# 3dhumangan/3DHumanGAN

Measured on AMD Instinct MI355X. Metric: generator images/sec at 512^2, higher is better.
Workload: dtype f32 in/out, f32 accumulate; contractions field f16x2 / synthesis f16x2 (x2 = f16 product + block-scaled fp6 cross terms, x3 = three f16/bf16 products); 1 GPU; BASELINE cfg 3: MAP3DBN512 generator-only forward, 512x512 out, 96x96 rays x 64 samples, hidden 256, batch 16/GPU, mixed, random-init weights, procedural SMPL-like pose; global_batch=16, parallelism=batch-sharded replicas x1 (no collective)

## Files before the change

### 3dhumangan_amd/_lib.py

```python
import ctypes as C
import os

_HERE = os.path.dirname(os.path.abspath(__file__))
LIB_PATH = os.path.join(_HERE, "csrc", "libh3d.so")

_lib = None


class H3DError(RuntimeError):
    pass


class FieldParams(C.Structure):
    _fields_ = [("w_coord", C.c_void_p), ("b_coord", C.c_void_p), ("w_geo", C.c_void_p), ("b_geo", C.c_void_p),
                ("w_film", C.c_void_p * 4), ("b_film", C.c_void_p * 4), ("w_sigma", C.c_void_p),
                ("b_sigma", C.c_void_p), ("w_color", C.c_void_p), ("b_color", C.c_void_p), ("w_rgb", C.c_void_p),
                ("b_rgb", C.c_void_p), ("w_feat", C.c_void_p), ("b_feat", C.c_void_p)]


_p, _i, _l, _f = C.c_void_p, C.c_int, C.c_int64, C.c_float
_SIGNATURES = {
    "h3d_version": (C.c_int, []),
    "h3d_last_error": (C.c_char_p, []),
    "h3d_device_info": (C.c_int, [C.POINTER(C.c_int), C.c_char_p, _i]),
    "h3d_ray_integrate": (C.c_int, [_p, _p, _p, _p, _p, _p, _l, _i, _i, _i, _i, _i, _p]),
    "h3d_ray_setup": (C.c_int, [_p, _p, _p, _p, _p, _p, _i, _i, _i, _i, _f, _f, _p]),
    "h3d_geo_features": (C.c_int, [_p, _p, _p, _p, _p, _p, _p, _i, _l, _i, _i, _i, _p]),
    "h3d_nearest_vertex": (C.c_int, [_p, _p, _p, _i, _l, _i, _p]),
    "h3d_mesh_sort_bytes": (C.c_int64, [_i, _i]),
    "h3d_mesh_sort": (C.c_int, [_p, _p, _i, _i, _p]),
    "h3d_geo_features_sorted": (C.c_int, [_p, _p, _p, _p, _p, _p, _p, _i, _l, _i, _i, _i, _p]),
    "h3d_nearest_vertex_sorted": (C.c_int, [_p, _p, _p, _i, _l, _i, _p]),
    "h3d_nearest_vertex_sorted_rays": (C.c_int, [_p, _p, _p, _i, _i, _i, _i, _i, _p]),
    "h3d_render_fused_x2_geo": (C.c_int, [_p] * 7 + [_i, _i] + [_p] * 8 + [_i, _i, _i, _i, _i, _f, _i, _i, _i, _p]),
    "h3d_render_fused_x3_geo": (C.c_int, [_p] * 7 + [_i, _i] + [_p] * 8 + [_i, _i, _i, _i, _i, _f, _i, _i, _i, _p]),
    "h3d_render_fused_x2_geo_ref": (C.c_int, [_p] * 7 + [_i, _i] + [_p] * 8 + [_i, _i, _i, _i, _i, _f, _i, _i, _i, _f, _f, _p, _p, _i, _p]),
    "h3d_render_fused_x3_geo_units": (C.c_int, [_p] * 7 + [_i, _i] + [_p] * 8 + [_i, _i, _i, _i, _i, _f, _i, _i, _i, _p, _p, _i, _p]),
    "h3d_field_pack_size": (C.c_int64, [_i, _i]),
    "h3d_field_pack": (C.c_int, [C.POINTER(FieldParams), _i, _i, _p]),
    "h3d_neural_field": (C.c_int, [_p, _p, _p, _p, _p, _p, _p, _i, _l, _i, _i, _i, _f, _p]),
    "h3d_render_fused": (C.c_int, [_p, _p, _p, _p, _p, _p, _p, _p, _p, _p, _p, _i, _i, _i, _i, _i, _i, _f, _i, _i,
                                   _i, _p]),
    "h3d_field_pack_x3_size": (C.c_int64, [_i, _i]),
    "h3d_field_pack_x3": (C.c_int, [C.POINTER(FieldParams), _i, _i, _p]),
    "h3d_field_pack_x3_device": (C.c_int, [C.POINTER(FieldParams), _i, _i, _p, _p]),
    "h3d_field_x3_layout": (C.c_int, [_i, _i, C.POINTER(C.c_int64), _i]),
    "h3d_neural_field_x3": (C.c_int, [_p, _p, _p, _p, _p, _p, _p, _i, _l, _i, _i, _i, _f, _p]),
    "h3d_render_fused_x3": (C.c_int, [_p, _p, _p, _p, _p, _p, _p, _p, _p, _p, _p, _i, _i, _i, _i, _i, _i, _f, _i,
                                      _i, _i, _p]),
    "h3d_conv_x3_tiling": (C.c_int, [_i, _i, C.POINTER(C.c_int)]),
    "h3d_conv_x3_pack": (C.c_int, [_p, _p, _i, _i, _i, _i, _p]),
    "h3d_conv_x3_pack_f16": (C.c_int, [_p, _p, _i, _i, _i, _i, _p]),
# ... 172 lines not shown
```

### 3dhumangan_amd/csrc/field_x3.hip

```cpp
#include "x3_common.hpp"
#include "field_pack.hpp"
#include "composite.hpp"
#include <string.h>
#include <math.h>
#include <stdio.h>
#include <algorithm>
#include <type_traits>

using namespace h3d;

namespace {

typedef F16::vec8 half8;
typedef F16::vec2 half2v;
typedef float f32x2 __attribute__((ext_vector_type(2)));

constexpr float kSA = 1.f;
constexpr float kSIn = 64.f;
constexpr int kLookF = 2;
constexpr int kValuF2 = 0;
constexpr int kValuF = 4;

enum { ST_COORD = 0, ST_GEO, ST_FILM0, ST_FILM1, ST_FILM2, ST_FILM3, ST_COLOR, ST_COUNT };
enum { W_COORD = 0, W_F0A, W_GEO, W_F0B, W_F1, W_F2, W_F3, W_COLOR, W_FEAT, W_COUNT };
// ... 53 lines not shown
    int Hd, F, geo_stride, S, clamp_mode, last_back, white_back;
    int R, log2S;
    int n_groups;
    float input_scaler;
    LayoutX3 L;
    const int* nn_index;
    const float* joints;
    const float* vertices;
    const float* tpose;
    const float* vertex_ik;
    int V, legacy_mode;
    int* ref_list;
    int* ref_count;
    int ref_cap, ref_mode;
    float ref_eps, ref_scale;
};

constexpr int kHeadPad = 64;
constexpr int kJointRows = 40;

__device__ __forceinline__ unsigned split2_act(float a, float b, unsigned& lo) {
    const half2v h2 = __builtin_convertvector(f32x2{a, b}, half2v);
    const float fa = (float)h2.x, fb = (float)h2.y;
    float la, lb;
    asm("v_sub_f32 %0, %1, %2" : "=v"(la) : "v"(a), "v"(fa));
    asm("v_sub_f32 %0, %1, %2" : "=v"(lb) : "v"(b), "v"(fb));
    lo = __builtin_bit_cast(unsigned, __builtin_convertvector(f32x2{la, lb}, half2v));
    return __builtin_bit_cast(unsigned, h2);
}

// ... 133 lines not shown
        const half8 tail[1] = {xl[KS]};
        gemm_x2_roll<NT, KS, KS3, 2 * NT + 1, NT, SWAP, kLookF, kValuF2, ZERO>(dst, xh, b6, tail, ring, hook, pre);
    } else {
        gemm_x3_roll<F16, NT, KSG, 2 * NT + 1, SWAP, kLookF, kValuF, ZERO>(dst, xh, xl, ring, hook);
    }
}

template <int NT, int KSG, typename RING, typename NEXT>
__device__ __forceinline__ void input_layer(f32x16 (&dst)[NT], const half8 (&ih)[2], const half8 (&il)[2], RING& ring, NEXT& next) {
    gemm_x3_roll<F16, NT, KSG, 2, false, kLookF, kValuF, true>(dst, ih, il, ring, [&](auto gc) __attribute__((always_inline)) {
        next_tile0<NT / 2, KSG - 1, decltype(gc)::value>(next);
    });
}


constexpr int kRingX2 = 8;

template <int NT, bool FUSED, bool X2, bool GEOIN = false>
__global__ __launch_bounds__(256, 1) void field_x3_kernel(Args A) {
    constexpr int KS = 2 * NT;
    extern __shared__ __attribute__((aligned(16))) float smem[];
    const LayoutX3& L = A.L;
    const int HdP = L.HdP;
    float* tab0 = smem;
    float* tfeat0 = tab0 + ST_COUNT * 2 * HdP;
    float* scratch = tfeat0 + HdP;
    float* joint0 = scratch + 4 * 64;
    unsigned char* head0 = reinterpret_cast<unsigned char*>(joint0 + (GEOIN ? kJointRows * 4 : 0));
    unsigned char* ring_lds = head0 + 4 * ((X2 ? 3 : 2) * KS * 32 + kHeadPad);

    const int t = threadIdx.x, lane = t & 63;
    const int wave = __builtin_amdgcn_readfirstlane(t >> 6);
    const int m = lane & 31, h = lane >> 5;
    const int b = blockIdx.y;
// ... 49 lines not shown
    __syncthreads();

    const float* __restrict__ head_inv = reinterpret_cast<const float*>(A.blob + L.head_inv);
    const float* __restrict__ head_b = reinterpret_cast<const float*>(A.blob + L.head_b);
    float inv_f = invs[W_FEAT];
    float hi0 = head_inv[0], hi1 = head_inv[1], hi2 = head_inv[2], hi3 = head_inv[3];
    float hb0 = head_b[0], hb1 = head_b[1], hb2 = head_b[2], hb3 = head_b[3];
    asm volatile("" : "+v"(inv_f), "+v"(hi0), "+v"(hi1), "+v"(hi2), "+v"(hi3), "+v"(hb0), "+v"(hb1), "+v"(hb2), "+v"(hb3));
    float* wl_lds = scratch + wave * 64;

    const int unit = FUSED ? (S > 32 ? S : 32) : 32;
    const int steps = unit / 32;
    const int seglen = FUSED ? (S < 32 ? S : 32) : 32;
    typedef typename std::conditional<X2, WeightRing<NT, kRingX2, 1>, WeightRing<NT>>::type Ring;
    Ring ring;
    ring.init(A.blob + L.w[0], ring_lds, L.stages, wave, lane);
    int n_groups = A.n_groups;
    if constexpr (FUSED) {
        if (A.ref_mode == 2) n_groups = (ref_units + 3) >> 2;
    }
    asm volatile("" : "+s"(n_groups));
    int ref_mode = FUSED ? A.ref_mode : 0;
    float ref_eps = A.ref_eps, ref_scale = A.ref_scale;
    typedef __attribute__((address_space(1))) int* gi32;
    gi32 ref_list = (gi32)A.ref_list + (int64_t)b * A.ref_cap, ref_count = (gi32)A.ref_count + b;
    int ref_cap = A.ref_cap;
    asm volatile("" : "+v"(ref_mode), "+v"(ref_eps), "+v"(ref_scale), "+v"(ref_list), "+v"(ref_count), "+v"(ref_cap));
    typedef const __attribute__((address_space(1))) float* gcf;
    typedef __attribute__((address_space(1))) float* gf;
    typedef const __attribute__((address_space(1))) int* gci;
    gcf a_points = (gcf)A.points, a_geo = (gcf)A.geo, a_dirs = (gcf)A.dirs, a_z = (gcf)A.z_vals, a_noise = (gcf)A.noise;
    gf a_feats = (gf)A.feats, a_depth = (gf)A.depth, a_weights = (gf)A.weights, a_out = (gf)A.out;
    gci a_nn = (gci)A.nn_index;
    gcf a_vik = (gcf)A.vertex_ik, a_tpose = (gcf)A.tpose, a_verts = (gcf)A.vertices;
    asm volatile("" : "+v"(a_points), "+v"(a_geo), "+v"(a_dirs), "+v"(a_z), "+v"(a_noise), "+v"(a_feats), "+v"(a_depth),
                      "+v"(a_weights), "+v"(a_out));
    if constexpr (GEOIN) asm volatile("" : "+v"(a_nn), "+v"(a_vik), "+v"(a_tpose), "+v"(a_verts));

#pragma unroll 1
    for (int ug = blockIdx.x; ug < n_groups; ug += gridDim.x) {
    int64_t uidx = (int64_t)ug * 4 + wave;
    if constexpr (FUSED) {
        if (ref_mode == 2) {
            const int slot = ug * 4 + wave;
            uidx = slot < ref_units ? (int64_t)__builtin_amdgcn_readfirstlane(ref_list[slot < ref_units ? slot : 0]) : N;
        }
    }
    const int64_t u0 = uidx * unit;
    const int64_t unit_ray = (int64_t)b * A.R + uidx;
    float smax = 0.f;
    auto ray_of = [&](int64_t nn) -> int64_t { return A.log2S < 0 ? unit_ray : (int64_t)b * A.R + (nn >> A.log2S); };

    RayCarry carry;
    float rgbacc = 0.f;
    float rayacc[NT];
#pragma unroll
    for (int i = 0; i < NT; ++i) rayacc[i] = 0.f;

    f32x16 X[NT], Y[NT];

    for (int si = 0; si < steps; ++si) {
        const int64_t n0 = u0 + (int64_t)si * 32;
        const int64_t n = n0 + m;
        const bool ok = n < N;
        const int64_t gi = (int64_t)b * N + (ok ? n : N - 1);
        const bool last_step = si == steps - 1;
        int opaque = 0;
        asm volatile("" : "+s"(opaque));
        const float* tab = tab0 + opaque;
// ... 118 lines not shown
            if (ok && h == 0) a_weights[gi] = w;
            if (h == 0) { wl_lds[m] = w; wl_lds[32 + m] = bg; }
            if (ref_mode == 1 && last_step) {
                float rmax = smax;
                for (int off = 1; off < seglen; off <<= 1) rmax = fmaxf(rmax, __shfl_xor(rmax, off, 32));
                const bool ill = last_abs >= 0.f && last_abs <= ref_eps * fmaxf(rmax, ref_scale);
                if (__any(ill)) {
                    if (lane == 0) {
                        const int slot = __hip_atomic_fetch_add(ref_count, 1, __ATOMIC_RELAXED, __HIP_MEMORY_SCOPE_AGENT);
                        if (slot < ref_cap) ref_list[slot] = (int)uidx;
                    }
                }
            }
        }

        layer<NT, KS, true, true, true, X2>(Y, xh, xl, b6, ring, p_col, none, hacc, head_lds, lane);
        pin_agpr<NT>(Y);
        float rgb[3];
        {
            const float c0 = __shfl(hacc[1], m, 64), c1 = __shfl(hacc[2], m, 64), c2 = __shfl(hacc[3], m, 64);
            rgb[0] = 1.f / (1.f + expf(-(c0 * hi1 + hb1)));
            rgb[1] = 1.f / (1.f + expf(-(c1 * hi2 + hb2)));
            rgb[2] = 1.f / (1.f + expf(-(c2 * hi3 + hb3)));
        }
        f32x16 (&acc)[NT] = Y;
        if (!FUSED) {
            if (ok && h == 0) {
                a_out[gi * (F + 4) + 0] = rgb[0];
                a_out[gi * (F + 4) + 1] = rgb[1];
                a_out[gi * (F + 4) + 2] = rgb[2];
            }
// ... 26 lines not shown
                    const int64_t ray = ray_of(n);
                    a_feats[ray * C + sl] = mine + (A.white_back ? bg : 0.f);
                }
            }
            __builtin_amdgcn_fence(__ATOMIC_RELEASE, "wavefront");
            __builtin_amdgcn_wave_barrier();
            float wr[16], wsum[4];
#pragma unroll
            for (int rg = 0; rg < 4; ++rg) {
                const f32x4 w4 = ld4(wl_lds + rg * 8 + 4 * h);
                wr[rg * 4 + 0] = w4.x; wr[rg * 4 + 1] = w4.y; wr[rg * 4 + 2] = w4.z; wr[rg * 4 + 3] = w4.w;
                wsum[rg] = (w4.x + w4.y) + (w4.z + w4.w);
            }
            const float wtot = (wsum[0] + wsum[1]) + (wsum[2] + wsum[3]);
            const float back = A.white_back ? wl_lds[32] : 0.f;
            gf fout = a_feats + ray_of(n0) * C + 3 + m;
            gf frg[4];
            float brg[4];
            bool okrg[4];
#pragma unroll
            for (int rg = 0; rg < 4; ++rg) {
                const int64_t n_first = n0 + rg * 8;
                okrg[rg] = h == 0 && n_first < N;
                frg[rg] = a_feats + ray_of(okrg[rg] ? n_first : n0) * C + 3 + m;
                brg[rg] = A.white_back ? wl_lds[32 + rg * 8] : 0.f;
            }
            const bool store_ray = last_step && h == 0 && n0 < N;
            const int g8 = S >> 3;
            const bool long_rays = S >= 32;
#pragma unroll
            for (int nt = 0; nt < NT; ++nt) {
                const int nn = nt * 32 + m;
                const bool okn = nn < F;
                const float bias = tfeat[okn ? nn : 0];
                pin1(acc[nt]);
                float s4[4];
#pragma unroll
                for (int rg = 0; rg < 4; ++rg) {
                    float s = acc[nt][rg * 4 + 0] * wr[rg * 4 + 0];
                    s = fmaf(acc[nt][rg * 4 + 1], wr[rg * 4 + 1], s);
                    s = fmaf(acc[nt][rg * 4 + 2], wr[rg * 4 + 2], s);
                    s4[rg] = fmaf(acc[nt][rg * 4 + 3], wr[rg * 4 + 3], s);
                }
                if (long_rays) {
                    float tot = fmaf((s4[0] + s4[1]) + (s4[2] + s4[3]), inv_f, bias * wtot);
                    tot += __shfl_xor(tot, 32, 64);
                    rayacc[nt] += tot;
                    if (store_ray && okn) fout[nt * 32] = rayacc[nt] + back;
                } else {
#pragma unroll
                    for (int rg = 0; rg < 4; ++rg) {
                        if (rg % g8 != 0) continue;
                        float sv = fmaf(s4[rg], inv_f, bias * wsum[rg]);
                        if (g8 == 2) sv += fmaf(s4[rg + 1 < 4 ? rg + 1 : 3], inv_f, bias * wsum[rg + 1 < 4 ? rg + 1 : 3]);
                        sv += __shfl_xor(sv, 32, 64);
                        if (okn && okrg[rg]) frg[rg][nt * 32] = sv + brg[rg];
                    }
                }
                __builtin_amdgcn_sched_barrier(0);
            }
            __builtin_amdgcn_wave_barrier();
        }
    }
    }
    ring.drain();
}

size_t lds_bytes(const LayoutX3& L, bool geoin = false) {
    return sizeof(float) * ((size_t)ST_COUNT * 2 * L.HdP + L.HdP + 4 * 64 + (geoin ? kJointRows * 4 : 0)) +
           (size_t)4 * (L.head_planes * L.KS * 32 + kHeadPad) + (L.head_planes == 3 ? kRingX2 : kWeightRingDepth) * (size_t)L.NT * 2048;
}

template <int NT, bool FUSED, bool X2, bool GEOIN = false>
int launch_one(Args A, int B, int64_t groups, hipStream_t st) {
    H3D_ALLOW_MAX_LDS((field_x3_kernel<NT, FUSED, X2, GEOIN>));
    A.n_groups = (int)groups;
    int64_t per_sample = h3d::persistent_wgs(groups, B, 4);
    if (A.ref_mode == 2) per_sample = std::max<int64_t>(1, std::min<int64_t>((A.ref_cap + 3) / 4, 8));
    h3d::pre_launch();
    hipLaunchKernelGGL((field_x3_kernel<NT, FUSED, X2, GEOIN>), dim3((unsigned)per_sample, (unsigned)B), dim3(256), lds_bytes(A.L, GEOIN), st, A);
    return h3d::launch_status(FUSED ? (X2 ? "h3d_render_fused_x2" : "h3d_render_fused_x3") : (X2 ? "h3d_neural_field_x2" : "h3d_neural_field_x3"));
}

template <bool FUSED>
int launch(const Args& A, int B, int64_t groups, hipStream_t st) {
    if constexpr (FUSED) {
        if (A.nn_index) {
            const bool x2 = A.L.head_planes == 3;
            if (A.L.NT == 4) return x2 ? launch_one<4, true, true, true>(A, B, groups, st) : launch_one<4, true, false, true>(A, B, groups, st);
            if (A.L.NT == 8) return x2 ? launch_one<8, true, true, true>(A, B, groups, st) : launch_one<8, true, false, true>(A, B, groups, st);
        }
    }
    if (A.L.head_planes == 3) {
        switch (A.L.NT) {
            case 4: return launch_one<4, FUSED, true>(A, B, groups, st);
            case 8: return launch_one<8, FUSED, true>(A, B, groups, st);
            default: break;
        }
    }
    switch (A.L.NT) {
        case 4: return launch_one<4, FUSED, false>(A, B, groups, st);
        case 8: return launch_one<8, FUSED, false>(A, B, groups, st);
        default:
// ... 258 lines not shown
    const float *joints, *vertices, *tpose, *vertex_ik;
    int V, legacy_mode;
};
struct RefIn {
    int mode;
    float eps, scale;
    int* list;
    int* count;
    int cap;
};

static int render_fused_x(bool x2, const void* packed, const float* points, const float* geo, const float* dirs,
                          const float* freq, const float* phase, const float* z_vals, const float* noise,
                          float* feats, float* depth, float* weights, int B, int R, int S, int Hd, int F,
                          int geo_stride, float input_scaler, int clamp_mode, int last_back, int white_back,
                          h3d_stream_t stream, const GeoIn* gin = nullptr, const RefIn* ref = nullptr) {
    const int64_t N = (int64_t)R * S;
    if (ref) {
        H3D_REQUIRE(ref->list && ref->count && ref->cap >= 1 && ref->cap <= 65536, "h3d_render_fused_x*: refinement list / count / cap=%d", ref->cap);
        H3D_REQUIRE(ref->mode == 2 || (ref->eps >= 0.f && ref->scale >= 0.f), "h3d_render_fused_x2_*_ref: eps and scale must be >= 0");
    }
    if (gin) {
        H3D_REQUIRE(gin->nn_index && gin->joints && gin->vertices && gin->tpose && gin->vertex_ik, "h3d_render_fused_x*_geo: null pointer");
        H3D_REQUIRE(gin->V >= 1 && h3d::aligned16(gin->vertex_ik), "h3d_render_fused_x*_geo: V=%d, vertex_ik must be 16-byte aligned", gin->V);
        geo = points;
        geo_stride = 31;
    }
    int rc = check_x3(packed, points, geo, freq, phase, B, N, Hd, F, geo_stride);
    if (rc) return rc;
    H3D_REQUIRE(z_vals && feats && depth && weights, "h3d_render_fused_x3: null pointer");
    H3D_REQUIRE(clamp_mode == 0 || clamp_mode == 1, "h3d_render_fused_x3: clamp_mode must be 0 (relu) or 1 (softplus)");
    H3D_REQUIRE(R >= 0 && S >= 1, "h3d_render_fused_x3: bad R=%d S=%d", R, S);
    const bool ok_s = (S >= 8 && S <= 32 && (S & (S - 1)) == 0) || (S > 32 && S % 32 == 0);
    if (!ok_s) {
        h3d::set_error("h3d_render_fused_x3: S=%d unsupported (needs 8, 16, 32 or a multiple of 32)", S);
        return H3D_EUNSUPPORTED;
    }
    if (B == 0 || N == 0) return H3D_OK;
    Args A{};
    A.blob = static_cast<const unsigned char*>(packed);
    A.points = points; A.geo = geo; A.dirs = dirs; A.freq = freq; A.phase = phase;
    A.z_vals = z_vals; A.noise = noise; A.feats = feats; A.depth = depth; A.weights = weights;
    A.N = N; A.Hd = Hd; A.F = F; A.geo_stride = geo_stride; A.S = S; A.input_scaler = input_scaler;
    A.clamp_mode = clamp_mode; A.last_back = last_back; A.white_back = white_back;
    A.R = R;
    A.log2S = -1;
    if (S <= 32) { A.log2S = 0; while ((1 << A.log2S) < S) ++A.log2S; }
    A.L = make_layout(Hd, F, x2);
    if (gin) {
        A.nn_index = gin->nn_index; A.joints = gin->joints; A.vertices = gin->vertices; A.tpose = gin->tpose;
        A.vertex_ik = gin->vertex_ik; A.V = gin->V; A.legacy_mode = gin->legacy_mode;
    }
    const int unit = S > 32 ? S : 32;
    const int64_t units = (N + unit - 1) / unit;
    const int64_t groups = (units + 3) / 4;
    H3D_REQUIRE(groups < (int64_t(1) << 31), "h3d_render_fused_x3: too many rays");
    if (ref) {
        A.ref_mode = ref->mode; A.ref_eps = ref->eps; A.ref_scale = ref->scale; A.ref_list = ref->list; A.ref_count = ref->count;
        A.ref_cap = ref->cap;
// ... 55 lines not shown
    return render_fused_x(true, packed, points, nullptr, dirs, freq, phase, z_vals, noise, feats, depth, weights, B, R, S, Hd, F, 31,
                          input_scaler, clamp_mode, last_back, white_back, stream, &g, &r);
}
extern "C" int h3d_render_fused_x3_geo_units(const void* packed, const float* points, const int32_t* nn_index, const float* joints,
                                             const float* vertices, const float* tpose_vertices, const float* vertex_ik, int V,
                                             int legacy_mode, const float* dirs, const float* freq, const float* phase,
                                             const float* z_vals, const float* noise, float* feats, float* depth, float* weights,
                                             int B, int R, int S, int Hd, int F, float input_scaler, int clamp_mode, int last_back,
                                             int white_back, const int32_t* ref_list, const int32_t* ref_count, int ref_cap,
                                             h3d_stream_t stream) {
    const GeoIn g{nn_index, joints, vertices, tpose_vertices, vertex_ik, V, legacy_mode};
    const RefIn r{2, 0.f, 0.f, const_cast<int32_t*>(ref_list), const_cast<int32_t*>(ref_count), ref_cap};
    return render_fused_x(false, packed, points, nullptr, dirs, freq, phase, z_vals, noise, feats, depth, weights, B, R, S, Hd, F, 31,
                          input_scaler, clamp_mode, last_back, white_back, stream, &g, &r);
}
```

### 3dhumangan_amd/lib/generators/map3d_generator.py

```python
import math
import os

import torch
import torch.nn as nn

from ... import _lib
from ..._stages import stage
from ..components import smpl
from ..components.ops.bias_act import bias_act
from . import volume_rendering as vr
from .differentiable import synthesis_forward
from .modsynth_pack import ModSynthesisPlan
from .style_input_pack import StyleInputPlan
from .synthesis_pack import SynthesisPlan


def normalize_2nd_moment(x, dim=1, eps=1e-8):
    return x * (x.square().mean(dim=dim, keepdim=True) + eps).rsqrt()


def _consume_camera_rng(sample_dist, batch, device):
    if sample_dist in ("uniform", "spherical_uniform"):
        torch.rand((batch, 1), device=device), torch.rand((batch, 1), device=device)
    elif sample_dist in ("normal", "gaussian"):
# ... 394 lines not shown
            feats, depths, weights = self._render_hierarchical(freq, phase, mesh, pts, z_vals, frame, S if fine_steps is None else int(fine_steps),
                                                               engine, lock_view_dependence, scaler, integ, nerf_noise, noise_coarse, fine_u, noise)
        else:
            noise = _integration_noise(noise, (B, R, S, 1), nerf_noise, dev)
            with stage(self, "geo_features"):
                if route == "fused_geo":
                    vik = smpl.vertex_inverse_transforms(c["fk_matrices"], c["lbs_weights"])
                    nn_index = smpl.nearest_vertex(pts, c["vertices"], ray_shape=(render_height, render_width, S))
                else:
                    geo = self.get_geo_features(pts, *mesh)
            dirs = None if lock_view_dependence else vr.ray_directions_world(focals, c["cam2world_matrices"], res, S)
            if route == "fused_geo":
                with stage(self, "render_fused"):
                    feats, depths, weights = nf.render_geo(pts, freq, phase, nn_index, *mesh[:3], vik, dirs, z_vals, S,
                                                           legacy_mode=self.legacy_mode, input_scaler=scaler, noise=noise,
                                                           precision=engine, **integ)
            elif route == "fused":
                with stage(self, "render_fused"):
                    feats, depths, weights = nf.render(pts, freq, phase, geo, dirs, z_vals, S, input_scaler=scaler, noise=noise,
                                                       precision=engine, **integ)
            else:
                with stage(self, "neural_field"):
                    field = nf(pts, freq, phase, geo, dirs, input_scaler=scaler, differentiable=differentiable, precision=engine)
                with stage(self, "ray_integrate"):
                    feats, depths, weights = vr.ray_integration(field.reshape(B, R, S, -1), z_vals, noise_std=0, noise=noise,
                                                                consume_rng=False, **integ)
        rgb_render = (feats[..., :3] * 2 - 1).reshape(B, render_height, render_width, 3).permute(0, 3, 1, 2)
        return rgb_render, feats[..., 3:], depths, weights, None

    def _render_hierarchical(self, freq, phase, mesh, pts, z_vals, frame, Sf, engine, lock_view_dependence, scaler, integ, nerf_noise,
                             noise_coarse, fine_u, noise):
# ... 178 lines not shown
```

### 3dhumangan_amd/lib/implicit_funcitions/modulated.py

```python
import ctypes
import math
import os
from typing import NamedTuple, Optional

import torch
import torch.nn as nn

from ... import _lib
from ..generators.volume_rendering import _CLAMP


class _Engine(NamedTuple):
    name: str
    pack_size: str
    pack: str
    device_pack: Optional[str]
    field: str
    render: str
    render_geo: Optional[str]
    tile: int
    tier: tuple


_ENGINES = {e.name: e for e in (
# ... 176 lines not shown
        pts, dirs, fr, ph, (z, nz, feats, depth, weights, mode) = self._prepare(input, ray_directions, frequencies, phase_shifts,
                                                                                 z_vals, num_steps, noise, clamp_mode)
        geo = geo_feature.contiguous().float()
        B, R, S = z.shape
        blob = self.packed_weights(pts.device, precision)
        rc = getattr(_lib.load(), eng.render)(_lib.ptr(blob), _lib.ptr(pts), _lib.ptr(geo), _lib.ptr(dirs), _lib.ptr(fr), _lib.ptr(ph),
                                              _lib.ptr(z), _lib.ptr(nz), _lib.ptr(feats), _lib.ptr(depth), _lib.ptr(weights), B, R, S,
                                              self.hidden_dim, self.feature_dim, geo.shape[-1], float(input_scaler), mode,
                                              int(bool(last_back)), int(bool(white_back)), *eng.tier, _lib.stream_handle())
        _lib.check(rc, "h3d_render_fused")
        return feats, depth, weights

    @torch.no_grad()
    def render_geo(self, input, frequencies, phase_shifts, nn_index, skeletons, vertices, tpose_vertices, vertex_ik,
                   ray_directions, z_vals, num_steps, legacy_mode=False, input_scaler=1., noise=None, clamp_mode="relu",
                   last_back=False, white_back=False, precision=None):
        _lib.need_cuda(input, frequencies, phase_shifts, nn_index, skeletons, vertices, tpose_vertices, vertex_ik,
                       ray_directions, z_vals, noise)
        eng = self._engine(precision)
        if eng.render_geo is None:
            raise ValueError(f"field engine {eng.name} has no fused render with in-kernel geometry")
        B, N, _ = input.shape
        idx = nn_index.contiguous()
        if idx.dtype != torch.int32 or tuple(idx.shape) != (B, N):
            raise ValueError("nn_index must be int32 [B, N]")
        sk, vt = skeletons.contiguous().float(), vertices.contiguous().float()
        tv, vik = tpose_vertices.contiguous().float(), vertex_ik.contiguous().float()
        if sk.shape[1:] != (24, 3) or vik.shape[1:] != (vt.shape[1], 16) or tv.shape != vt.shape:
            raise ValueError("skeletons [B,24,3], vertices / tpose_vertices [B,V,3], vertex_ik [B,V,16] expected")
        pts, dirs, fr, ph, (z, nz, feats, depth, weights, mode) = self._prepare(input, ray_directions, frequencies, phase_shifts,
                                                                                 z_vals, num_steps, noise, clamp_mode)
        _, R, S = z.shape
        blob = self.packed_weights(pts.device, precision)
        lib = _lib.load()
        common = lambda b: (_lib.ptr(b), _lib.ptr(pts), _lib.ptr(idx), _lib.ptr(sk), _lib.ptr(vt), _lib.ptr(tv), _lib.ptr(vik),
                            vt.shape[1], int(bool(legacy_mode)), _lib.ptr(dirs), _lib.ptr(fr), _lib.ptr(ph), _lib.ptr(z), _lib.ptr(nz),
                            _lib.ptr(feats), _lib.ptr(depth), _lib.ptr(weights), B, R, S, self.hidden_dim, self.feature_dim,
                            float(input_scaler), mode, int(bool(last_back)), int(bool(white_back)))
        if eng.name == "f16x2" and self.refine_last_sample:
            cap = self.refine_capacity
            buf = self._refine_buf
            if buf is None or buf[0].device != pts.device or buf[0].shape != (B, cap):
                buf = (torch.zeros(B, cap, dtype=torch.int32, device=pts.device), torch.zeros(B, dtype=torch.int32, device=pts.device))
                self._refine_buf = buf
            blob3 = self.packed_weights(pts.device, "f16x3")
            scale = self._sigma_scale(pts.device)
            rc = lib.h3d_render_fused_x2_geo_ref(*common(blob), float(self.refine_eps), scale, _lib.ptr(buf[0]), _lib.ptr(buf[1]), cap,
                                                 _lib.stream_handle())
            rc = rc or lib.h3d_render_fused_x3_geo_units(*common(blob3), _lib.ptr(buf[0]), _lib.ptr(buf[1]), cap, _lib.stream_handle())
        else:
            rc = getattr(lib, eng.render_geo)(*common(blob), _lib.stream_handle())
        _lib.check(rc, "h3d_render_fused_geo")
        return feats, depth, weights

    def _sigma_scale(self, device):
        w = self.sigma_layer.weight
        key = (w.data_ptr(), w._version, str(device))
        if self._sigma_scale_cache is None or self._sigma_scale_cache[0] != key:
            self._sigma_scale_cache = (key, float(w.detach().float().norm()))
        return self._sigma_scale_cache[1]

    def refined_units(self):
        return None if self._refine_buf is None else self._refine_buf[1]
```

### include/h3d.h

```cpp
#ifndef H3D_H
#define H3D_H

#include <stdint.h>

#ifdef __cplusplus
extern "C" {
#endif

#define H3D_VERSION 101

#define H3D_OK            0
#define H3D_EINVAL       -1
#define H3D_EUNSUPPORTED -2
#define H3D_ELAUNCH      -3

typedef void* h3d_stream_t;

int h3d_version(void);
const char* h3d_last_error(void);
int h3d_device_info(int* n_cu, char* name, int name_len);

int h3d_ray_integrate(const float* field, const float* z_vals, const float* noise,
                      float* feats, float* depth, float* weights,
                      int64_t n_rays, int S, int C,
// ... 139 lines not shown
int h3d_render_fused_x2_geo_ref(const void* packed, const float* points, const int32_t* nn_index, const float* joints,
                                const float* vertices, const float* tpose_vertices, const float* vertex_ik, int V,
                                int legacy_mode, const float* dirs, const float* freq, const float* phase,
                                const float* z_vals, const float* noise, float* feats, float* depth, float* weights,
                                int B, int R, int S, int Hd, int F, float input_scaler, int clamp_mode, int last_back,
                                int white_back, float ref_eps, float ref_scale, int32_t* ref_list, int32_t* ref_count,
                                int ref_cap, h3d_stream_t stream);
int h3d_render_fused_x3_geo_units(const void* packed, const float* points, const int32_t* nn_index, const float* joints,
                                  const float* vertices, const float* tpose_vertices, const float* vertex_ik, int V,
                                  int legacy_mode, const float* dirs, const float* freq, const float* phase,
                                  const float* z_vals, const float* noise, float* feats, float* depth, float* weights,
                                  int B, int R, int S, int Hd, int F, float input_scaler, int clamp_mode, int last_back,
                                  int white_back, const int32_t* ref_list, const int32_t* ref_count, int ref_cap,
                                  h3d_stream_t stream);

int64_t h3d_field_pack_x3t_size(int Hd, int F);
int h3d_field_pack_x3t(const h3d_field_params* p, int Hd, int F, void* blob );
int h3d_field_pack_x2t(const h3d_field_params* p, int Hd, int F, void* blob );
int h3d_field_x3t_layout(int Hd, int F, int64_t* out, int n_out);
int h3d_neural_field_x3t(const void* packed, const float* points, const float* geo, const float* dirs,
                         const float* freq, const float* phase, float* out,
                         int B, int64_t N, int Hd, int F, int geo_stride, float input_scaler,
                         h3d_stream_t stream);
int h3d_render_fused_x3t(const void* packed, const float* points, const float* geo, const float* dirs,
                         const float* freq, const float* phase, const float* z_vals, const float* noise,
                         float* feats, float* depth, float* weights,
                         int B, int R, int S, int Hd, int F, int geo_stride, float input_scaler,
                         int clamp_mode, int last_back, int white_back, h3d_stream_t stream);
int h3d_neural_field_x3t_tier(const void* packed, const float* points, const float* geo, const float* dirs,
                              const float* freq, const float* phase, float* out,
// ... 223 lines not shown
```

Measured before the change: 356.8 images/s.

## Composite hidden states per ray and apply feature head once per ray

Adds hidden-output variants of the fused geometry render kernels. Instead of running the final feature linear layer for every sample, they alpha-composite the pre-head hidden activations along each ray into a workspace, using identity-select MFMAs. A new per-ray kernel then applies the feature head, including bias scaled by total weight and the background term, producing the output features. This removes the per-sample feature GEMM. In exchange it adds a workspace round-trip, an extra launch, and a dependence on the head being linear in the hidden state.

```diff
diff --git a/3dhumangan_amd/_lib.py b/3dhumangan_amd/_lib.py
--- a/3dhumangan_amd/_lib.py
+++ b/3dhumangan_amd/_lib.py
@@ -36,6 +36,12 @@
     "h3d_render_fused_x3_geo": (C.c_int, [_p] * 7 + [_i, _i] + [_p] * 8 + [_i, _i, _i, _i, _i, _f, _i, _i, _i, _p]),
     "h3d_render_fused_x2_geo_ref": (C.c_int, [_p] * 7 + [_i, _i] + [_p] * 8 + [_i, _i, _i, _i, _i, _f, _i, _i, _i, _f, _f, _p, _p, _i, _p]),
     "h3d_render_fused_x3_geo_units": (C.c_int, [_p] * 7 + [_i, _i] + [_p] * 8 + [_i, _i, _i, _i, _i, _f, _i, _i, _i, _p, _p, _i, _p]),
+    "h3d_render_fused_x2_geo_hidden": (C.c_int, [_p] * 7 + [_i, _i] + [_p] * 8 + [_i, _i, _i, _i, _i, _f, _i, _i, _i, _p, _p]),
+    "h3d_render_fused_x3_geo_hidden": (C.c_int, [_p] * 7 + [_i, _i] + [_p] * 8 + [_i, _i, _i, _i, _i, _f, _i, _i, _i, _p, _p]),
+    "h3d_render_fused_x2_geo_ref_hidden": (C.c_int, [_p] * 7 + [_i, _i] + [_p] * 8 + [_i, _i, _i, _i, _i, _f, _i, _i, _i, _f, _f, _p, _p, _i, _p,
+                                                     _p]),
+    "h3d_render_fused_x3_geo_units_hidden": (C.c_int, [_p] * 7 + [_i, _i] + [_p] * 8 + [_i, _i, _i, _i, _i, _f, _i, _i, _i, _p, _p, _i, _p, _p]),
+    "h3d_ray_feature_head": (C.c_int, [_p, _p, _p, _l, _i, _i, _p]),
     "h3d_field_pack_size": (C.c_int64, [_i, _i]),
     "h3d_field_pack": (C.c_int, [C.POINTER(FieldParams), _i, _i, _p]),
     "h3d_neural_field": (C.c_int, [_p, _p, _p, _p, _p, _p, _p, _i, _l, _i, _i, _i, _f, _p]),
diff --git a/3dhumangan_amd/csrc/field_x3.hip b/3dhumangan_amd/csrc/field_x3.hip
--- a/3dhumangan_amd/csrc/field_x3.hip
+++ b/3dhumangan_amd/csrc/field_x3.hip
@@ -91,6 +91,7 @@
     int* ref_count;
     int ref_cap, ref_mode;
     float ref_eps, ref_scale;
+    float* hidden_ws;
 };
 
 constexpr int kHeadPad = 64;
@@ -254,10 +255,46 @@
 }
 
 
+template <int NT, bool X2, typename PROD>
+__device__ __forceinline__ void hidden_tail(f32x16 (&dst)[NT], half8 (&xh)[2 * NT + 1], half8 (&xl)[2 * NT + 1], PROD& prod, f32x16& hacc,
+                                            const unsigned char* head_lds, int lane, const half8 (&selh)[2], const half8 (&sell)[2]) {
+    constexpr int KS = 2 * NT, PL = X2 ? 3 : 2;
+    const lds_ptr hbase = lane_base(head_lds, (lane & 3) * (PL * KS * 32 + kHeadPad) + (lane >> 5) * 16);
+    static_for<0, NT>([&](auto tc) __attribute__((always_inline)) {
+        constexpr int t = decltype(tc)::value;
+        const f32x16 zero = {0.f, 0.f, 0.f, 0.f, 0.f, 0.f, 0.f, 0.f, 0.f, 0.f, 0.f, 0.f, 0.f, 0.f, 0.f, 0.f};
+        u32x4 hwh[2], hwl[2], hws[2];
+#pragma unroll
+        for (int j = 0; j < 2; ++j) {
+            hwh[j] = lds_ld<u32x4>(hbase + (2 * t + j) * 32);
+            hwl[j] = lds_ld<u32x4>(hbase + (KS + 2 * t + j) * 32);
+            if constexpr (X2) hws[j] = lds_ld<u32x4>(hbase + (2 * KS + 2 * t + j) * 32);
+        }
+        if constexpr (t + 1 < NT) {
+            static_for<0, 8>([&](auto c) __attribute__((always_inline)) { prod.template chunk<t + 1, decltype(c)::value>(); });
+        }
+#pragma unroll
+        for (int j = 0; j < 2; ++j) {
+            const int s = 2 * t + j;
+            const half8 ah = __builtin_bit_cast(half8, hwh[j]), al = __builtin_bit_cast(half8, hwl[j]);
+            hacc = F16::mfma(ah, xh[s], s == 0 ? zero : hacc);
+            hacc = F16::mfma(X2 ? __builtin_bit_cast(half8, hws[j]) : ah, xl[s], hacc);
+            hacc = F16::mfma(al, xh[s], hacc);
+        }
+        dst[t] = F16::mfma(xh[2 * t], selh[0], zero);
+        dst[t] = F16::mfma(xl[2 * t], sell[0], dst[t]);
+        dst[t] = F16::mfma(xh[2 * t + 1], selh[1], dst[t]);
+        dst[t] = F16::mfma(xl[2 * t + 1], sell[1], dst[t]);
+        asm volatile("" : "+a"(dst[t]));
+        __builtin_amdgcn_sched_barrier(0);
+    });
+}
+
 constexpr int kRingX2 = 8;
 
-template <int NT, bool FUSED, bool X2, bool GEOIN = false>
+template <int NT, bool FUSED, bool X2, bool GEOIN = false, bool HIDDEN = false>
 __global__ __launch_bounds__(256, 1) void field_x3_kernel(Args A) {
+    static_assert(!HIDDEN || (FUSED && GEOIN), "the composited-hidden variant exists for the fused kernels with in-kernel geometry");
     constexpr int KS = 2 * NT;
     extern __shared__ __attribute__((aligned(16))) float smem[];
     const LayoutX3& L = A.L;
@@ -337,7 +374,7 @@
     const int seglen = FUSED ? (S < 32 ? S : 32) : 32;
     typedef typename std::conditional<X2, WeightRing<NT, kRingX2, 1>, WeightRing<NT>>::type Ring;
     Ring ring;
-    ring.init(A.blob + L.w[0], ring_lds, L.stages, wave, lane);
+    ring.init(A.blob + L.w[0], ring_lds, HIDDEN ? L.stages - KS : L.stages, wave, lane);
     int n_groups = A.n_groups;
     if constexpr (FUSED) {
         if (A.ref_mode == 2) n_groups = (ref_units + 3) >> 2;
@@ -359,6 +396,26 @@
     asm volatile("" : "+v"(a_points), "+v"(a_geo), "+v"(a_dirs), "+v"(a_z), "+v"(a_noise), "+v"(a_feats), "+v"(a_depth),
                       "+v"(a_weights), "+v"(a_out));
     if constexpr (GEOIN) asm volatile("" : "+v"(a_nn), "+v"(a_vik), "+v"(a_tpose), "+v"(a_verts));
+    gf a_ws = (gf)A.hidden_ws;
+    half8 selh[2], sell[2];
+    if constexpr (HIDDEN) {
+        asm volatile("" : "+v"(a_ws));
+        const int e0 = (m & 3) + 4 * ((m >> 3) & 1);
+#pragma unroll
+        for (int j = 0; j < 2; ++j) {
+            const bool on = h == ((m >> 2) & 1) && j == (m >> 4);
+            u32x4 one = {0u, 0u, 0u, 0u}, inv = {0u, 0u, 0u, 0u};
+#pragma unroll
+            for (int wd = 0; wd < 4; ++wd) {
+                const bool hit = on && wd == (e0 >> 1);
+                one[wd] = hit ? 0x3C00u << (16 * (e0 & 1)) : 0u;
+                inv[wd] = hit ? (X2 ? 0x0C00u : 0x3C00u) << (16 * (e0 & 1)) : 0u;
+            }
+            asm volatile("" : "+v"(one), "+v"(inv));
+            selh[j] = __builtin_bit_cast(half8, one);
+            sell[j] = __builtin_bit_cast(half8, inv);
+        }
+    }
 
 #pragma unroll 1
     for (int ug = blockIdx.x; ug < n_groups; ug += gridDim.x) {
@@ -375,7 +432,7 @@
     auto ray_of = [&](int64_t nn) -> int64_t { return A.log2S < 0 ? unit_ray : (int64_t)b * A.R + (nn >> A.log2S); };
 
     RayCarry carry;
-    float rgbacc = 0.f;
+    float rgbacc = 0.f, wacc = 0.f;
     float rayacc[NT];
 #pragma unroll
     for (int i = 0; i < NT; ++i) rayacc[i] = 0.f;
@@ -524,7 +581,8 @@
             }
         }
 
-        layer<NT, KS, true, true, true, X2>(Y, xh, xl, b6, ring, p_col, none, hacc, head_lds, lane);
+        if constexpr (HIDDEN) hidden_tail<NT, X2>(Y, xh, xl, p_col, hacc, head_lds, lane, selh, sell);
+        else layer<NT, KS, true, true, true, X2>(Y, xh, xl, b6, ring, p_col, none, hacc, head_lds, lane);
         pin_agpr<NT>(Y);
         float rgb[3];
         {
@@ -581,7 +639,8 @@
             }
             const float wtot = (wsum[0] + wsum[1]) + (wsum[2] + wsum[3]);
             const float back = A.white_back ? wl_lds[32] : 0.f;
-            gf fout = a_feats + ray_of(n0) * C + 3 + m;
+            const int WS = HdP + 4;
+            gf fout = HIDDEN ? a_ws + ray_of(n0) * WS + m : a_feats + ray_of(n0) * C + 3 + m;
             gf frg[4];
             float brg[4];
             bool okrg[4];
@@ -589,7 +648,7 @@
             for (int rg = 0; rg < 4; ++rg) {
                 const int64_t n_first = n0 + rg * 8;
                 okrg[rg] = h == 0 && n_first < N;
-                frg[rg] = a_feats + ray_of(okrg[rg] ? n_first : n0) * C + 3 + m;
+                frg[rg] = HIDDEN ? a_ws + ray_of(okrg[rg] ? n_first : n0) * WS + m : a_feats + ray_of(okrg[rg] ? n_first : n0) * C + 3 + m;
                 brg[rg] = A.white_back ? wl_lds[32 + rg * 8] : 0.f;
             }
             const bool store_ray = last_step && h == 0 && n0 < N;
@@ -598,8 +657,8 @@
 #pragma unroll
             for (int nt = 0; nt < NT; ++nt) {
                 const int nn = nt * 32 + m;
-                const bool okn = nn < F;
-                const float bias = tfeat[okn ? nn : 0];
+                const bool okn = HIDDEN || nn < F;
+                const float bias = HIDDEN ? 0.f : tfeat[nn < F ? nn : 0];
                 pin1(acc[nt]);
                 float s4[4];
 #pragma unroll
@@ -610,21 +669,43 @@
                     s4[rg] = fmaf(acc[nt][rg * 4 + 3], wr[rg * 4 + 3], s);
                 }
                 if (long_rays) {
-                    float tot = fmaf((s4[0] + s4[1]) + (s4[2] + s4[3]), inv_f, bias * wtot);
+                    float tot = (s4[0] + s4[1]) + (s4[2] + s4[3]);
+                    if constexpr (!HIDDEN) tot = fmaf(tot, inv_f, bias * wtot);
                     tot += __shfl_xor(tot, 32, 64);
                     rayacc[nt] += tot;
-                    if (store_ray && okn) fout[nt * 32] = rayacc[nt] + back;
+                    if (store_ray && okn) fout[nt * 32] = HIDDEN ? rayacc[nt] : rayacc[nt] + back;
                 } else {
 #pragma unroll
                     for (int rg = 0; rg < 4; ++rg) {
                         if (rg % g8 != 0) continue;
-                        float sv = fmaf(s4[rg], inv_f, bias * wsum[rg]);
-                        if (g8 == 2) sv += fmaf(s4[rg + 1 < 4 ? rg + 1 : 3], inv_f, bias * wsum[rg + 1 < 4 ? rg + 1 : 3]);
+                        float sv;
+                        if constexpr (HIDDEN) {
+                            sv = s4[rg];
+                            if (g8 == 2) sv += s4[rg + 1 < 4 ? rg + 1 : 3];
+                        } else {
+                            sv = fmaf(s4[rg], inv_f, bias * wsum[rg]);
+                            if (g8 == 2) sv += fmaf(s4[rg + 1 < 4 ? rg + 1 : 3], inv_f, bias * wsum[rg + 1 < 4 ? rg + 1 : 3]);
+                        }
                         sv += __shfl_xor(sv, 32, 64);
-                        if (okn && okrg[rg]) frg[rg][nt * 32] = sv + brg[rg];
+                        if (okn && okrg[rg]) frg[rg][nt * 32] = HIDDEN ? sv : sv + brg[rg];
                     }
                 }
                 __builtin_amdgcn_sched_barrier(0);
+            }
+            if constexpr (HIDDEN) {
+                if (long_rays) {
+                    wacc += wtot + __shfl_xor(wtot, 32, 64);
+                    if (store_ray && m < 4) fout[HdP] = m == 0 ? wacc : m == 1 ? back : 0.f;
+                } else {
+#pragma unroll
+                    for (int rg = 0; rg < 4; ++rg) {
+                        if (rg % g8 != 0) continue;
+                        float wv = wsum[rg];
+                        if (g8 == 2) wv += wsum[rg + 1 < 4 ? rg + 1 : 3];
+                        wv += __shfl_xor(wv, 32, 64);
+                        if (okrg[rg] && m < 4) frg[rg][HdP] = m == 0 ? wv : m == 1 ? brg[rg] : 0.f;
+                    }
+                }
             }
             __builtin_amdgcn_wave_barrier();
         }
@@ -638,14 +719,14 @@
            (size_t)4 * (L.head_planes * L.KS * 32 + kHeadPad) + (L.head_planes == 3 ? kRingX2 : kWeightRingDepth) * (size_t)L.NT * 2048;
 }
 
-template <int NT, bool FUSED, bool X2, bool GEOIN = false>
+template <int NT, bool FUSED, bool X2, bool GEOIN = false, bool HIDDEN = false>
 int launch_one(Args A, int B, int64_t groups, hipStream_t st) {
-    H3D_ALLOW_MAX_LDS((field_x3_kernel<NT, FUSED, X2, GEOIN>));
+    H3D_ALLOW_MAX_LDS((field_x3_kernel<NT, FUSED, X2, GEOIN, HIDDEN>));
     A.n_groups = (int)groups;
     int64_t per_sample = h3d::persistent_wgs(groups, B, 4);
     if (A.ref_mode == 2) per_sample = std::max<int64_t>(1, std::min<int64_t>((A.ref_cap + 3) / 4, 8));
     h3d::pre_launch();
-    hipLaunchKernelGGL((field_x3_kernel<NT, FUSED, X2, GEOIN>), dim3((unsigned)per_sample, (unsigned)B), dim3(256), lds_bytes(A.L, GEOIN), st, A);
+    hipLaunchKernelGGL((field_x3_kernel<NT, FUSED, X2, GEOIN, HIDDEN>), dim3((unsigned)per_sample, (unsigned)B), dim3(256), lds_bytes(A.L, GEOIN), st, A);
     return h3d::launch_status(FUSED ? (X2 ? "h3d_render_fused_x2" : "h3d_render_fused_x3") : (X2 ? "h3d_neural_field_x2" : "h3d_neural_field_x3"));
 }
 
@@ -654,6 +735,10 @@
     if constexpr (FUSED) {
         if (A.nn_index) {
             const bool x2 = A.L.head_planes == 3;
+            if (A.hidden_ws) {
+                if (A.L.NT == 4) return x2 ? launch_one<4, true, true, true, true>(A, B, groups, st) : launch_one<4, true, false, true, true>(A, B, groups, st);
+                if (A.L.NT == 8) return x2 ? launch_one<8, true, true, true, true>(A, B, groups, st) : launch_one<8, true, false, true, true>(A, B, groups, st);
+            }
             if (A.L.NT == 4) return x2 ? launch_one<4, true, true, true>(A, B, groups, st) : launch_one<4, true, false, true>(A, B, groups, st);
             if (A.L.NT == 8) return x2 ? launch_one<8, true, true, true>(A, B, groups, st) : launch_one<8, true, false, true>(A, B, groups, st);
         }
@@ -942,8 +1027,10 @@
                           const float* freq, const float* phase, const float* z_vals, const float* noise,
                           float* feats, float* depth, float* weights, int B, int R, int S, int Hd, int F,
                           int geo_stride, float input_scaler, int clamp_mode, int last_back, int white_back,
-                          h3d_stream_t stream, const GeoIn* gin = nullptr, const RefIn* ref = nullptr) {
+                          h3d_stream_t stream, const GeoIn* gin = nullptr, const RefIn* ref = nullptr, float* hidden_ws = nullptr,
+                          bool hidden = false) {
     const int64_t N = (int64_t)R * S;
+    if (hidden) H3D_REQUIRE(gin && hidden_ws && h3d::aligned16(hidden_ws), "h3d_render_fused_x*_hidden: hidden_ws must be a 16-byte aligned buffer");
     if (ref) {
         H3D_REQUIRE(ref->list && ref->count && ref->cap >= 1 && ref->cap <= 65536, "h3d_render_fused_x*: refinement list / count / cap=%d", ref->cap);
         H3D_REQUIRE(ref->mode == 2 || (ref->eps >= 0.f && ref->scale >= 0.f), "h3d_render_fused_x2_*_ref: eps and scale must be >= 0");
@@ -971,6 +1058,7 @@
     A.z_vals = z_vals; A.noise = noise; A.feats = feats; A.depth = depth; A.weights = weights;
     A.N = N; A.Hd = Hd; A.F = F; A.geo_stride = geo_stride; A.S = S; A.input_scaler = input_scaler;
     A.clamp_mode = clamp_mode; A.last_back = last_back; A.white_back = white_back;
+    A.hidden_ws = hidden ? hidden_ws : nullptr;
     A.R = R;
     A.log2S = -1;
     if (S <= 32) { A.log2S = 0; while ((1 << A.log2S) < S) ++A.log2S; }
@@ -1056,3 +1144,155 @@
     return render_fused_x(false, packed, points, nullptr, dirs, freq, phase, z_vals, noise, feats, depth, weights, B, R, S, Hd, F, 31,
                           input_scaler, clamp_mode, last_back, white_back, stream, &g, &r);
 }
+
+extern "C" int h3d_render_fused_x2_geo_hidden(const void* packed, const float* points, const int32_t* nn_index, const float* joints,
+                                              const float* vertices, const float* tpose_vertices, const float* vertex_ik, int V,
+                                              int legacy_mode, const float* dirs, const float* freq, const float* phase,
+                                              const float* z_vals, const float* noise, float* feats, float* depth, float* weights,
+                                              int B, int R, int S, int Hd, int F, float input_scaler, int clamp_mode, int last_back,
+                                              int white_back, float* hidden_ws, h3d_stream_t stream) {
+    const GeoIn g{nn_index, joints, vertices, tpose_vertices, vertex_ik, V, legacy_mode};
+    return render_fused_x(true, packed, points, nullptr, dirs, freq, phase, z_vals, noise, feats, depth, weights, B, R, S, Hd, F, 31,
+                          input_scaler, clamp_mode, last_back, white_back, stream, &g, nullptr, hidden_ws, true);
+}
+extern "C" int h3d_render_fused_x3_geo_hidden(const void* packed, const float* points, const int32_t* nn_index, const float* joints,
+                                              const float* vertices, const float* tpose_vertices, const float* vertex_ik, int V,
+                                              int legacy_mode, const float* dirs, const float* freq, const float* phase,
+                                              const float* z_vals, const float* noise, float* feats, float* depth, float* weights,
+                                              int B, int R, int S, int Hd, int F, float input_scaler, int clamp_mode, int last_back,
+                                              int white_back, float* hidden_ws, h3d_stream_t stream) {
+    const GeoIn g{nn_index, joints, vertices, tpose_vertices, vertex_ik, V, legacy_mode};
+    return render_fused_x(false, packed, points, nullptr, dirs, freq, phase, z_vals, noise, feats, depth, weights, B, R, S, Hd, F, 31,
+                          input_scaler, clamp_mode, last_back, white_back, stream, &g, nullptr, hidden_ws, true);
+}
+extern "C" int h3d_render_fused_x2_geo_ref_hidden(const void* packed, const float* points, const int32_t* nn_index, const float* joints,
+                                                  const float* vertices, const float* tpose_vertices, const float* vertex_ik, int V,
+                                                  int legacy_mode, const float* dirs, const float* freq, const float* phase,
+                                                  const float* z_vals, const float* noise, float* feats, float* depth, float* weights,
+                                                  int B, int R, int S, int Hd, int F, float input_scaler, int clamp_mode, int last_back,
+                                                  int white_back, float ref_eps, float ref_scale, int32_t* ref_list, int32_t* ref_count,
+                                                  int ref_cap, float* hidden_ws, h3d_stream_t stream) {
+    const GeoIn g{nn_index, joints, vertices, tpose_vertices, vertex_ik, V, legacy_mode};
+    const RefIn r{1, ref_eps, ref_scale, ref_list, ref_count, ref_cap};
+    return render_fused_x(true, packed, points, nullptr, dirs, freq, phase, z_vals, noise, feats, depth, weights, B, R, S, Hd, F, 31,
+                          input_scaler, clamp_mode, last_back, white_back, stream, &g, &r, hidden_ws, true);
+}
+extern "C" int h3d_render_fused_x3_geo_units_hidden(const void* packed, const float* points, const int32_t* nn_index, const float* joints,
+                                                    const float* vertices, const float* tpose_vertices, const float* vertex_ik, int V,
+                                                    int legacy_mode, const float* dirs, const float* freq, const float* phase,
+                                                    const float* z_vals, const float* noise, float* feats, float* depth, float* weights,
+                                                    int B, int R, int S, int Hd, int F, float input_scaler, int clamp_mode, int last_back,
+                                                    int white_back, const int32_t* ref_list, const int32_t* ref_count, int ref_cap,
+                                                    float* hidden_ws, h3d_stream_t stream) {
+    const GeoIn g{nn_index, joints, vertices, tpose_vertices, vertex_ik, V, legacy_mode};
+    const RefIn r{2, 0.f, 0.f, const_cast<int32_t*>(ref_list), const_cast<int32_t*>(ref_count), ref_cap};
+    return render_fused_x(false, packed, points, nullptr, dirs, freq, phase, z_vals, noise, feats, depth, weights, B, R, S, Hd, F, 31,
+                          input_scaler, clamp_mode, last_back, white_back, stream, &g, &r, hidden_ws, true);
+}
+
+namespace {
+
+struct HeadArgs {
+    const unsigned char* blob;
+    const float* ws;
+    float* feats;
+    int64_t M;
+    int F, n_groups;
+    LayoutX3 L;
+};
+
+template <int NT>
+__global__ __launch_bounds__(256, 1) void ray_head_kernel(HeadArgs A) {
+    constexpr int KS = 2 * NT;
+    extern __shared__ __attribute__((aligned(16))) float smem[];
+    const LayoutX3& L = A.L;
+    const int HdP = L.HdP, F = A.F, WS = HdP + 4, C = F + 3;
+    float* tfeat = smem;
+    unsigned char* ring_lds = reinterpret_cast<unsigned char*>(smem + HdP);
+    const int t = threadIdx.x, lane = t & 63;
+    const int wave = __builtin_amdgcn_readfirstlane(t >> 6);
+    const int m = lane & 31, h = lane >> 5;
+    const float* __restrict__ bf = reinterpret_cast<const float*>(A.blob + L.b_feat);
+    for (int idx = t; idx < HdP; idx += 256) tfeat[idx] = idx < F ? bf[idx] : 0.f;
+    __syncthreads();
+    float inv_f = reinterpret_cast<const float*>(A.blob + L.inv_scale)[W_FEAT];
+    asm volatile("" : "+v"(inv_f));
+    typedef const __attribute__((address_space(1))) float* gcf;
+    typedef __attribute__((address_space(1))) float* gf;
+    typedef const __attribute__((address_space(1))) f32x4* gcf4;
+    gcf a_ws = (gcf)A.ws;
+    gf a_feats = (gf)A.feats;
+    const int64_t M = A.M;
+    WeightRing<NT> ring;
+    ring.init(A.blob + L.w[W_FEAT], ring_lds, KS, wave, lane);
+#pragma unroll 1
+    for (int ug = blockIdx.x; ug < A.n_groups; ug += gridDim.x) {
+        const int64_t r0 = (int64_t)ug * 128 + wave * 32;
+        const int64_t mine = r0 + m < M ? r0 + m : M - 1;
+        gcf c = a_ws + mine * WS + 4 * h;
+        half8 xh[KS], xl[KS];
+#pragma unroll
+        for (int ks = 0; ks < KS; ++ks) {
+            const f32x4 a = *reinterpret_cast<gcf4>(c + 32 * (ks / 2) + 16 * (ks & 1));
+            const f32x4 b = *reinterpret_cast<gcf4>(c + 32 * (ks / 2) + 16 * (ks & 1) + 8);
+            const float v[8] = {a.x, a.y, a.z, a.w, b.x, b.y, b.z, b.w};
+            split8(v, kSA, xh[ks], xl[ks]);
+        }
+        f32x16 acc[NT];
+        gemm_x3_roll<F16, NT, KS, KS, true, kLookF, 0, true>(acc, xh, xl, ring);
+        float sw[16], bk[16];
+        bool okr[16];
+#pragma unroll
+        for (int r = 0; r < 16; ++r) {
+            const int64_t row = r0 + (r >> 2) * 8 + 4 * h + (r & 3);
+            okr[r] = row < M;
+            gcf tl = a_ws + (okr[r] ? row : M - 1) * WS + HdP;
+            sw[r] = tl[0];
+            bk[r] = tl[1];
+        }
+#pragma unroll
+        for (int nt = 0; nt < NT; ++nt) {
+            const int nn = nt * 32 + m;
+            if (nn >= F) continue;
+            const float bias = tfeat[nn];
+#pragma unroll
+            for (int r = 0; r < 16; ++r) {
+                const int64_t row = r0 + (r >> 2) * 8 + 4 * h + (r & 3);
+                if (okr[r]) a_feats[row * C + 3 + nn] = fmaf(acc[nt][r], inv_f, bias * sw[r]) + bk[r];
+            }
+        }
+    }
+    ring.drain();
+}
+
+template <int NT>
+int launch_head(HeadArgs A, int64_t groups, hipStream_t st) {
+    H3D_ALLOW_MAX_LDS((ray_head_kernel<NT>));
+    A.n_groups = (int)groups;
+    const int64_t wgs = h3d::persistent_wgs(groups, 1, 2);
+    const size_t lds = sizeof(float) * (size_t)A.L.HdP + (size_t)kWeightRingDepth * A.L.NT * 2048;
+    h3d::pre_launch();
+    hipLaunchKernelGGL((ray_head_kernel<NT>), dim3((unsigned)wgs), dim3(256), lds, st, A);
+    return h3d::launch_status("h3d_ray_feature_head");
+}
+
+}
+
+extern "C" int h3d_ray_feature_head(const void* packed_x3, const float* hidden_ws, float* feats, int64_t M, int Hd, int F,
+                                    h3d_stream_t stream) {
+    H3D_REQUIRE(packed_x3 && hidden_ws && feats, "h3d_ray_feature_head: null pointer");
+    H3D_REQUIRE(h3d::aligned16(packed_x3) && h3d::aligned16(hidden_ws), "h3d_ray_feature_head: packed weights and hidden_ws must be 16-byte aligned");
+    H3D_REQUIRE(M >= 0 && Hd >= 1 && F >= 1, "h3d_ray_feature_head: bad M=%lld Hd=%d F=%d", (long long)M, Hd, F);
+    if (Hd > 256 || F > 256) {
+        h3d::set_error("h3d_ray_feature_head: widths up to 256 (got %d/%d)", Hd, F);
+        return H3D_EUNSUPPORTED;
+    }
+    if (M == 0) return H3D_OK;
+    HeadArgs A{};
+    A.blob = static_cast<const unsigned char*>(packed_x3);
+    A.ws = hidden_ws; A.feats = feats; A.M = M; A.F = F;
+    A.L = make_layout(Hd, F, false);
+    const int64_t groups = (M + 127) / 128;
+    H3D_REQUIRE(groups < (int64_t(1) << 31), "h3d_ray_feature_head: too many rows");
+    return A.L.NT == 4 ? launch_head<4>(A, groups, static_cast<hipStream_t>(stream)) : launch_head<8>(A, groups, static_cast<hipStream_t>(stream));
+}
diff --git a/3dhumangan_amd/lib/generators/map3d_generator.py b/3dhumangan_amd/lib/generators/map3d_generator.py
--- a/3dhumangan_amd/lib/generators/map3d_generator.py
+++ b/3dhumangan_amd/lib/generators/map3d_generator.py
@@ -432,7 +432,7 @@
                 with stage(self, "render_fused"):
                     feats, depths, weights = nf.render_geo(pts, freq, phase, nn_index, *mesh[:3], vik, dirs, z_vals, S,
                                                            legacy_mode=self.legacy_mode, input_scaler=scaler, noise=noise,
-                                                           precision=engine, **integ)
+                                                           precision=engine, per_ray_head=True, **integ)
             elif route == "fused":
                 with stage(self, "render_fused"):
                     feats, depths, weights = nf.render(pts, freq, phase, geo, dirs, z_vals, S, input_scaler=scaler, noise=noise,
diff --git a/3dhumangan_amd/lib/implicit_funcitions/modulated.py b/3dhumangan_amd/lib/implicit_funcitions/modulated.py
--- a/3dhumangan_amd/lib/implicit_funcitions/modulated.py
+++ b/3dhumangan_amd/lib/implicit_funcitions/modulated.py
@@ -214,7 +214,7 @@
     @torch.no_grad()
     def render_geo(self, input, frequencies, phase_shifts, nn_index, skeletons, vertices, tpose_vertices, vertex_ik,
                    ray_directions, z_vals, num_steps, legacy_mode=False, input_scaler=1., noise=None, clamp_mode="relu",
-                   last_back=False, white_back=False, precision=None):
+                   last_back=False, white_back=False, precision=None, per_ray_head=False):
         _lib.need_cuda(input, frequencies, phase_shifts, nn_index, skeletons, vertices, tpose_vertices, vertex_ik,
                        ray_directions, z_vals, noise)
         eng = self._engine(precision)
@@ -233,6 +233,12 @@
         _, R, S = z.shape
         blob = self.packed_weights(pts.device, precision)
         lib = _lib.load()
+        sfx, ws = "", None
+        if per_ray_head:
+            hdp = 128 if max(self.hidden_dim, self.feature_dim) <= 128 else 256
+            sfx, ws = "_hidden", torch.empty((B * R, hdp + 4), device=pts.device, dtype=torch.float32)
+            blob3 = self.packed_weights(pts.device, "f16x3")
+        tail = lambda *own: own + ((_lib.ptr(ws),) if per_ray_head else ()) + (_lib.stream_handle(),)
         common = lambda b: (_lib.ptr(b), _lib.ptr(pts), _lib.ptr(idx), _lib.ptr(sk), _lib.ptr(vt), _lib.ptr(tv), _lib.ptr(vik),
                             vt.shape[1], int(bool(legacy_mode)), _lib.ptr(dirs), _lib.ptr(fr), _lib.ptr(ph), _lib.ptr(z), _lib.ptr(nz),
                             _lib.ptr(feats), _lib.ptr(depth), _lib.ptr(weights), B, R, S, self.hidden_dim, self.feature_dim,
@@ -245,11 +251,14 @@
                 self._refine_buf = buf
             blob3 = self.packed_weights(pts.device, "f16x3")
             scale = self._sigma_scale(pts.device)
-            rc = lib.h3d_render_fused_x2_geo_ref(*common(blob), float(self.refine_eps), scale, _lib.ptr(buf[0]), _lib.ptr(buf[1]), cap,
-                                                 _lib.stream_handle())
-            rc = rc or lib.h3d_render_fused_x3_geo_units(*common(blob3), _lib.ptr(buf[0]), _lib.ptr(buf[1]), cap, _lib.stream_handle())
+            rc = getattr(lib, "h3d_render_fused_x2_geo_ref" + sfx)(*common(blob), *tail(float(self.refine_eps), scale, _lib.ptr(buf[0]),
+                                                                                       _lib.ptr(buf[1]), cap))
+            rc = rc or getattr(lib, "h3d_render_fused_x3_geo_units" + sfx)(*common(blob3), *tail(_lib.ptr(buf[0]), _lib.ptr(buf[1]), cap))
         else:
-            rc = getattr(lib, eng.render_geo)(*common(blob), _lib.stream_handle())
+            rc = getattr(lib, eng.render_geo + sfx)(*common(blob), *tail())
+        if per_ray_head:
+            rc = rc or lib.h3d_ray_feature_head(_lib.ptr(blob3), _lib.ptr(ws), _lib.ptr(feats), B * R, self.hidden_dim, self.feature_dim,
+                                                _lib.stream_handle())
         _lib.check(rc, "h3d_render_fused_geo")
         return feats, depth, weights
 
diff --git a/include/h3d.h b/include/h3d.h
--- a/include/h3d.h
+++ b/include/h3d.h
@@ -177,6 +177,35 @@
                                   int white_back, const int32_t* ref_list, const int32_t* ref_count, int ref_cap,
                                   h3d_stream_t stream);
 
+int h3d_render_fused_x2_geo_hidden(const void* packed, const float* points, const int32_t* nn_index, const float* joints,
+                                   const float* vertices, const float* tpose_vertices, const float* vertex_ik, int V,
+                                   int legacy_mode, const float* dirs, const float* freq, const float* phase,
+                                   const float* z_vals, const float* noise, float* feats, float* depth, float* weights,
+                                   int B, int R, int S, int Hd, int F, float input_scaler, int clamp_mode, int last_back,
+                                   int white_back, float* hidden_ws, h3d_stream_t stream);
+int h3d_render_fused_x3_geo_hidden(const void* packed, const float* points, const int32_t* nn_index, const float* joints,
+                                   const float* vertices, const float* tpose_vertices, const float* vertex_ik, int V,
+                                   int legacy_mode, const float* dirs, const float* freq, const float* phase,
+                                   const float* z_vals, const float* noise, float* feats, float* depth, float* weights,
+                                   int B, int R, int S, int Hd, int F, float input_scaler, int clamp_mode, int last_back,
+                                   int white_back, float* hidden_ws, h3d_stream_t stream);
+int h3d_render_fused_x2_geo_ref_hidden(const void* packed, const float* points, const int32_t* nn_index, const float* joints,
+                                       const float* vertices, const float* tpose_vertices, const float* vertex_ik, int V,
+                                       int legacy_mode, const float* dirs, const float* freq, const float* phase,
+                                       const float* z_vals, const float* noise, float* feats, float* depth, float* weights,
+                                       int B, int R, int S, int Hd, int F, float input_scaler, int clamp_mode, int last_back,
+                                       int white_back, float ref_eps, float ref_scale, int32_t* ref_list, int32_t* ref_count,
+                                       int ref_cap, float* hidden_ws, h3d_stream_t stream);
+int h3d_render_fused_x3_geo_units_hidden(const void* packed, const float* points, const int32_t* nn_index, const float* joints,
+                                         const float* vertices, const float* tpose_vertices, const float* vertex_ik, int V,
+                                         int legacy_mode, const float* dirs, const float* freq, const float* phase,
+                                         const float* z_vals, const float* noise, float* feats, float* depth, float* weights,
+                                         int B, int R, int S, int Hd, int F, float input_scaler, int clamp_mode, int last_back,
+                                         int white_back, const int32_t* ref_list, const int32_t* ref_count, int ref_cap,
+                                         float* hidden_ws, h3d_stream_t stream);
+int h3d_ray_feature_head(const void* packed_x3, const float* hidden_ws, float* feats, int64_t M, int Hd, int F,
+                         h3d_stream_t stream);
+
 int64_t h3d_field_pack_x3t_size(int Hd, int F);
 int h3d_field_pack_x3t(const h3d_field_params* p, int Hd, int F, void* blob );
 int h3d_field_pack_x2t(const h3d_field_params* p, int Hd, int F, void* blob );
```

Measured after the change: 363.0 images/s, median of 6. 1.02x the previous value.
